# richardbaihe/a3t

Hardware: AMD Instinct MI355X
Metric: mel-frames/sec (train) (higher is better)
Workload: dtype bf16; 1 GPU; VCTK A3T masked-mel train step: 6+6 Conformer blocks d=384 H=2 ff=1536(k3), B=32/GPU, T_mel=1000, T_phn=120, postnet 5x256x5, fwd+bwd+clip+Adam, dropout 0.2/0.2/0.2 + postnet 0.5 (recipe); global_batch=32, parallelism=dp1, params=100799808

## Files before the change

### a3t_amd/_lib.py

```python
import ctypes
import os
from ctypes import POINTER, c_char_p, c_float, c_int, c_int32, c_int64, c_void_p

import torch

HERE = os.path.dirname(os.path.abspath(__file__))
LIB_PATH = os.environ.get("A3T_LIB_PATH") or os.path.join(HERE, "lib", "liba3t_hip.so")

F32, BF16 = 0, 1
BF16X3 = 2
ACT_NONE, ACT_RELU, ACT_TANH, ACT_SWISH = 0, 1, 2, 3
ACC_STORE, ACC_ADD, ACC_ATOMIC, ACC_SOLE = 0, 1, 2, 3


class GemmDesc(ctypes.Structure):
    _fields_ = [
        ("A", c_void_p), ("B", c_void_p), ("C", c_void_p), ("bias", c_void_p), ("R", c_void_p), ("S", c_void_p),
        ("M", c_int32), ("N", c_int32), ("K", c_int32),
        ("a_rs", c_int64), ("a_cs", c_int64),
        ("b_rs", c_int64), ("b_cs", c_int64), ("b_ts", c_int64),
        ("c_rs", c_int64),
        ("batch", c_int32), ("batch_inner", c_int32),
        ("a_bs0", c_int64), ("a_bs1", c_int64), ("b_bs0", c_int64), ("b_bs1", c_int64),
        ("c_bs0", c_int64), ("c_bs1", c_int64),
        ("taps", c_int32), ("pad", c_int32), ("dil", c_int32), ("Tseq", c_int32), ("kshift", c_int32),
        ("alpha", c_float),
        ("act", c_int32), ("accumulate", c_int32), ("splitk", c_int32),
        ("a_dtype", c_int32), ("b_dtype", c_int32), ("c_dtype", c_int32), ("compute", c_int32),
        ("s_dtype", c_int32), ("colsum_slots", c_int32),
        ("colsum", c_void_p), ("colsum_bs1", c_int64), ("colsum_scale", c_float), ("drop_key", ctypes.c_uint32),
        ("drop_p", c_float), ("colsum_ss", c_int32),
        ("keep_out", c_void_p), ("keep_in", c_void_p),
        ("a_signmask", c_int32), ("keep_layout", c_int32),
        ("A2", c_void_p), ("B2", c_void_p), ("b2_cs", c_int64), ("b2_bs0", c_int64), ("b2_bs1", c_int64), ("colsum2", c_void_p),
        ("a2_rs", c_int64), ("a_unaligned", c_int32),
    ]


_P = c_void_p
_SIGS = {
    "a3t_gemm": [POINTER(GemmDesc), _P],
    "a3t_gemm_plan": [POINTER(GemmDesc), c_char_p, c_int],
    "a3t_layernorm_fwd": [_P, _P, _P, _P, c_int, _P, _P, c_int, c_int, c_float, _P],
    "a3t_layernorm_bwd": [_P, c_int, _P, _P, _P, _P, _P, _P, _P, _P, _P, _P, c_float, c_int, c_int, c_float,
                          ctypes.c_uint32, _P],
    "a3t_col_reduce": [_P, c_int, _P, _P, _P, _P, c_int, c_int, c_int64, c_int, _P],
    "a3t_f64_to_f32_add": [_P, _P, c_int, c_float, _P],
    "a3t_bn_act_fwd": [_P, _P, _P, _P, _P, _P, _P, _P, _P, c_int, c_int, c_int, c_float, c_float, c_int, c_int, _P],
    "a3t_bn_act_bwd_a": [_P, c_int, _P, _P, _P, _P, _P, _P, c_int, c_int, c_int, _P],
    "a3t_bn_act_bwd_b": [_P, c_int, _P, _P, _P, _P, _P, _P, _P, _P, _P, c_int, c_int, c_int, c_int, _P],
    "a3t_glu_dwconv_fwd": [_P, c_int, _P, _P, _P, c_int, _P, c_int, c_int, c_int, c_int, _P],
    "a3t_glu_dwconv_bwd": [_P, _P, c_int, _P, c_int, _P, _P, c_int, _P, _P, _P, c_int, c_int, c_int, c_int, _P],
    "a3t_add_pos_bias": [_P, _P, _P, _P, _P, c_int, c_int, c_int, _P],
    "a3t_add_pos_bias_bwd": [_P, _P, _P, c_int, c_int, c_int, _P],
    "a3t_relpos_softmax_fwd": [_P, _P, c_int, _P, _P, c_int, c_int, c_int, c_int, c_int64, c_int64, c_int64, c_float, _P,
                               c_float, ctypes.c_uint32, _P],
    "a3t_relpos_softmax_bwd": [_P, c_int, _P, c_int, _P, _P, c_int, c_int, c_int, c_int, c_int64, c_int64, c_int64, c_float, _P,
                               c_float, c_int64, c_int64, ctypes.c_uint32, _P, _P],
    "a3t_attn_fwd_train": [_P, _P, _P, _P, _P, _P, _P, _P, _P, _P, _P, c_int, c_int, c_int, c_int, c_int64, c_int64, c_int64,
                           c_int64, c_float, c_float, ctypes.c_uint32, _P, _P, _P],
    "a3t_attn_scale_rows": [_P, _P, _P, c_int, c_int, c_int, c_int, _P],
    "a3t_attn_bwd_ds": [_P, _P, _P, _P, _P, _P, _P, c_int, c_int, c_int, c_int, c_int64, c_int64, c_int64, c_int64, c_float,
                        c_float, ctypes.c_uint32, c_int, c_int64, _P],
    "a3t_attn_fwd": [_P, _P, _P, _P, _P, _P, _P, _P, c_int, c_int, c_int, c_int, c_int64, c_int64, c_int64, c_int64,
                     c_float, c_float, ctypes.c_uint32, _P, _P, _P],
    "a3t_pwg_block": [_P, _P, _P, _P, _P, _P, _P, _P, c_int, c_int, c_int, _P],
    "a3t_mask_fill": [_P, _P, _P, _P, c_int, c_int, c_int, _P],
    "a3t_embed_finish_fwd": [_P, _P, _P, _P, _P, _P, _P, c_int, c_int, c_int, c_int, c_float, c_float, ctypes.c_uint32,
                             _P, _P],
    "a3t_embed_finish_bwd": [_P, _P, _P, _P, _P, _P, _P, _P, c_int, c_int, c_int, c_int, c_int, c_int, c_float, c_float,
                             ctypes.c_uint32, _P],
    "a3t_scale": [_P, _P, c_int64, c_float, _P],
    "a3t_attn_fwd_plain": [_P, _P, _P, _P, _P, _P, c_int, c_int, c_int, c_int, c_int64, c_int64, c_int64, c_float, c_float,
                           ctypes.c_uint32, _P],
    "a3t_attn_fwd_train_plain": [_P, _P, _P, _P, _P, _P, _P, _P, _P, c_int, c_int, c_int, c_int, c_int64, c_int64, c_int64, c_float,
                                 c_float, ctypes.c_uint32, _P],
    "a3t_embed_finish_abs_fwd": [_P, _P, _P, _P, _P, _P, _P, _P, _P, _P, c_int, c_int, c_int, c_int, c_float, c_float,
                                 ctypes.c_uint32, _P, _P],
    "a3t_embed_finish_abs_bwd": [_P, _P, _P, _P, _P, _P, _P, _P, _P, _P, _P, _P, c_int, c_int, c_int, c_int, c_int, c_int,
                                 c_float, c_float, ctypes.c_uint32, _P],
    "a3t_embed_finish_abs_partials": [c_int, c_int, c_int, c_int],
    "a3t_scale_add_pos": [_P, _P, _P, c_int, c_int, c_int, c_float, c_float, ctypes.c_uint32, _P],
    "a3t_softmax_plain_fwd": [_P, c_int, _P, _P, c_int, c_int, c_int, c_int, c_int64, c_int64, c_float, _P, c_float,
                              ctypes.c_uint32, _P],
    "a3t_softmax_plain_bwd": [_P, c_int, _P, c_int, _P, c_int, c_int, c_int, c_int, c_int64, c_int64, c_int64, c_float, _P,
                              c_float, ctypes.c_uint32, _P, _P],
    "a3t_axpy": [_P, _P, c_int64, c_float, _P],
    "a3t_attn_bias_fold": [_P, c_int32, c_int32, _P, _P, _P, _P],
    "a3t_scale_dev": [_P, _P, c_int64, _P, _P],
    "a3t_slice_rows": [_P, _P, c_int, c_int, c_int, c_int, c_int, c_int, _P],
    "a3t_concat_rows": [_P, _P, _P, c_int, c_int, c_int, c_int, _P],
    "a3t_concat_rows_ragged": [_P, _P, _P, _P, _P, c_int, c_int, c_int, c_int, c_int64, c_int64, _P],
    "a3t_split_rows": [_P, _P, _P, c_int, c_int, c_int, c_int, _P],
    "a3t_cast_bf16": [_P, _P, c_int64, _P],
    "a3t_cast_bf16_conv_t": [_P, _P, _P, _P, c_int, c_int, c_int, c_int, _P],
    "a3t_split_bf16": [_P, _P, _P, c_int64, _P],
    "a3t_reflect_pad": [_P, _P, c_int, c_int, c_int, c_int, _P],
    "a3t_reflect_pad_ragged": [_P, _P, _P, c_int, c_int, c_int, c_int, _P],
    "a3t_stft_amp": [_P, _P, c_int64, c_int, c_int, _P],
    "a3t_logmel_finish": [_P, _P, c_int, c_int, c_int, _P],
    "a3t_mlm_loss": [_P, _P, _P, _P, _P, _P, _P, _P, c_int, c_int, c_int, c_float, _P],
    "a3t_mlm_loss_scratch_floats": [c_int],
    "a3t_sumsq": [_P, c_int64, _P, _P],
    "a3t_clip_adam": [_P, _P, _P, _P, _P, _P, c_int64, c_float, c_float, c_float, c_float, c_int, c_float, c_float,
                      _P],
    "a3t_clip_adam_noam": [_P, _P, _P, _P, _P, _P, c_int64, _P, c_float, c_float, c_float, c_float, c_float, c_float,
                           c_float, c_float, _P],
    "a3t_sgd_step": [_P, _P, c_int64, c_float, c_float, _P],
    "a3t_pwg_gate": [_P, _P, _P, c_int64, c_int, _P],
    "a3t_pwg_res_skip": [_P, _P, _P, c_int64, c_int, c_int, _P],
    "a3t_pwg_upsample": [_P, _P, _P, c_int64, c_int64, c_int, c_int, _P],
    "a3t_replicate_pad": [_P, _P, c_int64, c_int64, c_int, c_int, _P],
    "a3t_bias_act": [_P, _P, c_int64, c_int, c_int, c_float, _P],
    "a3t_replicate_pad_ragged": [_P, _P, _P, c_int64, c_int64, c_int, c_int, _P],
    "a3t_pwg_upsample_ragged": [_P, _P, _P, _P, c_int, c_int64, c_int64, c_int, c_int, _P],
    "a3t_zero_tail": [_P, _P, c_int, c_int64, c_int64, c_int, _P],
# ... 83 lines not shown
```

### a3t_amd/build.py

```python
import os
import subprocess
import sys
from concurrent.futures import ThreadPoolExecutor

HERE = os.path.dirname(os.path.abspath(__file__))
CSRC = os.path.join(HERE, "csrc")
LIBDIR = os.path.join(HERE, "lib")
LIB = os.path.join(LIBDIR, "liba3t_hip.so")
SOURCES = ["gemm.hip", "gemm_bf16.hip", "gemm_bf16_8p.hip", "gemm_bf16_tn.hip", "gemm_bf16_pn.hip", "gemm_bf16_tt.hip", "attn_fused.hip", "norm_reduce.hip", "convmod_attn.hip", "dwconv_vec.hip", "misc.hip", "pwg_fused.hip", "pwg_fused_f16.hip", "features.hip", "duration.hip", "fs2_tts.hip", "gst.hip", "hifigan.hip", "hifigan_f16.hip", "melgan.hip", "stylemelgan.hip"]
FLAGS = ["--offload-arch=gfx950", "-O3", "-std=c++17", "-fPIC", "-ffp-contract=off"] + os.environ.get("A3T_EXTRA_FLAGS", "").split()


WAVE_SOURCES = ("pwg_fused.hip", "pwg_fused_f16.hip", "hifigan.hip", "hifigan_f16.hip", "melgan.hip", "stylemelgan.hip")
RES_SOURCES = ("gemm_bf16.hip", "gemm_bf16_8p.hip", "gemm_bf16_tn.hip", "gemm_bf16_pn.hip", "gemm_bf16_tt.hip", "attn_fused.hip", "norm_reduce.hip") + WAVE_SOURCES
RES_FLAG = ["-Rpass-analysis=kernel-resource-usage"]


def _save_resources(report, path):
    import json
    import re
    cur, rows = None, {}
    for ln in report.splitlines():
        m = re.search(r"Function Name: (\S+)", ln)
        if m:
            cur = m.group(1)
            rows[cur] = {}
            continue
        m = re.search(r"remark:\s+([\w \[\]/]+?): (\d+)", ln)
        if m and cur:
            rows[cur][m.group(1).strip()] = int(m.group(2))
    with open(path, "w") as f:
        json.dump(rows, f, indent=1)


def _hipcc():
    for c in ("/opt/rocm/bin/hipcc", "hipcc"):
        if os.path.exists(c) or c == "hipcc":
            return c


def _stale(out, deps):
    if not os.path.exists(out):
        return True
    t = os.path.getmtime(out)
    return any(os.path.getmtime(d) > t for d in deps)


def build(force=False, verbose=True):
    os.makedirs(LIBDIR, exist_ok=True)
    hdrs = [os.path.join(os.path.dirname(HERE), "include", "a3t_hip.h")]
    hdrs += sorted(os.path.join(CSRC, h) for h in os.listdir(CSRC) if h.endswith(".h"))
    objs, jobs = [], []
    for s in SOURCES:
        src = os.path.join(CSRC, s)
        obj = os.path.join(LIBDIR, s.replace(".hip", ".o"))
        objs.append(obj)
        if force or _stale(obj, [src] + hdrs):
            jobs.append([_hipcc(), *FLAGS, "-c", src, "-o", obj] + (RES_FLAG if s in RES_SOURCES else []))

    def run(cmd):
        if verbose:
            print(" ".join(cmd), flush=True)
        if RES_FLAG[0] in cmd:
            r = subprocess.run(cmd, stderr=subprocess.PIPE, text=True)
            if r.returncode:
                sys.stderr.write(r.stderr)
                raise subprocess.CalledProcessError(r.returncode, cmd)
# ... 15 lines not shown
```

### a3t_amd/conformer.py

```python
import math
import os
import zlib
from dataclasses import dataclass

import torch

from . import ops
from ._lib import ACC_ADD, ACC_ATOMIC, ACC_STORE, ACT_RELU, ACT_SWISH, BF16, BF16X3, F32
from .config import A3TConfig
from .params import ParamStore
from .schedule import StepSchedule


def legacy_pe_table(c: A3TConfig) -> torch.Tensor:
    d = c.adim
    position = torch.arange(c.max_len - 1, -1, -1.0, dtype=torch.float32).unsqueeze(1)
    div = torch.exp(torch.arange(0, d, 2, dtype=torch.float32) * -(math.log(10000.0) / d))
    pe = torch.zeros(c.max_len, d)
    pe[:, 0::2] = torch.sin(position * div)
    pe[:, 1::2] = torch.cos(position * div)
    return pe


def score_chunks(lengths, heads, max_score_elems):
# ... 447 lines not shown
        if rs is not None:
            dctx_v = self._act(self._t("tmp.dctxs"), (M, d))
        signed = bool(self.sv.get(tag + ".signed"))
        adr = self._drop(c.attention_dropout_rate, tag + ".att") if (pdrop is not None or signed) else None
        regen = self.bf16 and adr is not None and T % 8 == 0 and T <= 2048
        ds_fused = (rs is not None and self.bf16 and self.opt.attn_bwd_ds and (adr is None or regen) and dk % 32 == 0 and dk <= 192
                    and dk != 160 and T % 8 == 0)
        zb = (H * T * T, T * T)
        assert ds_fused or not signed
        if not ds_fused:
            dpr = self.ws.get("tmp.ac", (B, H, T, T), sdt)
            ops.gemm(dctx, vv, dpr, T, T, dk, d, 1, 3 * d, 1, T, batch=B * H, batch_inner=H, a_bs=(T * d, dk),
                     b_bs=(T * 3 * d, dk), c_bs=zb, compute=cmp)
        fz = self.bf16
        gbq = gr[pre + ".bqkv"]
        S = self.colsum_slots
        sl = self._arena_slot("bwd32", tag + ".bsl", S * 4 * d) if fz else None
        csk = dict(colsum_bs1=dk, colsum_slots=S, colsum_ss=4 * d)
        make_q = qu is None
        if make_q:
            qu = self._act("tmp.qu", (M, d))
            qv = self._act(self._t("tmp.qv"), (M, d))

        def dv_gemm():
            if rs is not None:
                ops.attn_scale_rows(dctx, rs, dctx_v, B, H, T)
            ops.gemm(pdrop if pdrop is not None else probs, dctx_v, dvv, T, dk, T, 1, T, 1, d, 3 * d,
                     batch=B * H, batch_inner=H, a_bs=zb, b_bs=(T * d, dk), c_bs=(T * 3 * d, dk),
                     compute=cmp, colsum=sl[3 * d:] if fz else None, a_signmask=signed,
                     alpha=1.0 / (1.0 - adr[0]) if signed else 1.0, **csk)
            if make_q:
                ops.add_pos_bias(qkv, p[pre + ".u"], p[pre + ".v"], qu, qv)
        qv_ready = self._side(dv_gemm, want_event=make_q, urgent=True)
        zbd = zb
        dual = ds_fused and fz and self.opt.attn_dq_dual and ops.gemm_tt_supported(T, dk, T, B * H)
        dview = ds_fused and fz and self.opt.attn_dbd_view
        if dview:
            bsv = T + T * T
            flat = self.ws.get(self._t("tmp.dsv"), (B * H * bsv,), torch.bfloat16, zero_once=True)
            ds, dbd = flat[T:], flat[1:]
            zbd = (H * bsv, bsv)
        elif self.bf16:
            ds = self.ws.get("tmp.ds16", (B, H, T, T), torch.bfloat16)
            dbd = self.ws.get(self._t("tmp.dbd16"), (B, H, T, T), torch.bfloat16)
        else:
            ds = dpr
            dbd = self.ws.get(self._t("tmp.dbd"), (B, H, T, T), sdt)
        if ds_fused:
            ops.attn_bwd_ds(dctx, ctx, qkv, probs, rs, ds, None if dview else dbd, B, H, T, scale, drop=adr or (0.0, 0),
                            signed_probs=signed, ds_bs=zbd[1] if dview else 0)
        else:
            ops.relpos_softmax_bwd(probs, dpr, ds, dbd, B, H, T, scale, probs_drop=None if regen else pdrop,
                                   drop_p=adr[0] if adr else 0.0, drop_key=adr[1] if regen else 0, rowscale=rs)
        def pos_weight_grad():
            if qv_ready is not None and self.side is not None:
                qv_ready.wait_on(self.side)
            dP = self._arena_slot("bwd32", tag + ".dP", T * d).view(T, d)
            ops.gemm(dbd, qv, dP, T, dk, T, 1, T + 1 if dview else T, 1, d, d, batch=B * H, batch_inner=H, a_bs=zbd, b_bs=(T * d, dk),
                     c_bs=(0, dk), acc=ACC_ATOMIC, compute=cmp, a_view=dview)
            if self.bf16:
                dP16 = self.ws.get("tmp.dP16", (T, d), torch.bfloat16)
                ops.cast_bf16(dP, dP16)
                dP = dP16
            ops.linear_bwd_weight(dP, pos, gr[pre + ".wpos"], compute=cmp)
        self._side(pos_weight_grad)
        dq_acc = fz
        dqu = dqkv if dq_acc else self._act("tmp.dqu", (M, d))
        dqv = dqkv if dq_acc else self._act("tmp.dqv", (M, d))
        ldq, cbq = (3 * d, (T * 3 * d, dk)) if dq_acc else (d, (T * d, dk))
        if dual:
            ops.gemm(ds, kk, dqkv, T, dk, T, T, 1, 1, 3 * d, ldq, batch=B * H, batch_inner=H, a_bs=zbd,
                     b_bs=(T * 3 * d, dk), c_bs=cbq, compute=cmp, colsum=sl,
                     second=(dbd, P, d, (0, dk), sl[d:]) + ((T + 1,) if dview else ()), **csk)
        else:
            ops.gemm(ds, kk, dqu, T, dk, T, T, 1, 1, 3 * d, ldq, batch=B * H, batch_inner=H, a_bs=zbd,
                     b_bs=(T * 3 * d, dk), c_bs=cbq, compute=cmp, colsum=sl if fz else None, **csk)
        dk_fn = lambda: ops.gemm(ds, qu, dkk, T, dk, T, 1, T, 1, d, 3 * d, batch=B * H, batch_inner=H,
                                 a_bs=zbd, b_bs=(T * d, dk), c_bs=(T * 3 * d, dk), compute=cmp,
                                 colsum=sl[2 * d:] if fz else None, **csk)
        if self.opt.attn_dk_main and dual and self.side is not None and make_q and qv_ready is not None:
            qv_ready.wait_on(torch.cuda.current_stream())
            dk_fn()
            dk_done = None
        else:
            dk_done = self._side(dk_fn, want_event=True, urgent=True)
        if not dual:
            ops.gemm(dbd, P, dqv, T, dk, T, T + 1 if dview else T, 1, 1, d, ldq, batch=B * H, batch_inner=H, a_bs=zbd, b_bs=(0, dk),
                     c_bs=cbq, acc=ACC_ADD if dq_acc else ACC_STORE, compute=cmp, colsum=sl[d:] if fz else None, a_view=dview, **csk)
        if not dq_acc:
            ops.add_pos_bias_bwd(dqu, dqv, dqkv)
        if dk_done is not None:
            dk_done.wait_on(torch.cuda.current_stream())
        if fz:
            self._side(
                lambda: ops.attn_bias_fold(sl, S, d, gr[pre + ".u"], gr[pre + ".v"], gbq))
        else:
            self._bias_grad(dqu, gr[pre + ".u"])
            self._bias_grad(dqv, gr[pre + ".v"])
            self._bias_grad(dqkv, gbq)
        self._lin_wgrad(dqkv, y, gr[pre + ".wqkv"])
        dy = self._act("tmp.dy", (M, d))
        self._lin_dgrad(dqkv, pre + ".wqkv", dy)
        self._pre_ln(ga, g, g16)
        self._ln_bwd(tag + ".ln", dy, pre + ".ln", g, g, g16, nb, nxt)
        self._sub_end()
        return g

    def _bn_fwd(self, tag, z, pre, bufpre, act, out):
        p, b = self.store.p, self.store.buf
# ... 210 lines not shown
```

### a3t_amd/ops.py

```python
import ctypes
import os

import torch

from . import _lib as L
from ._lib import ACC_ADD, ACC_ATOMIC, ACC_SOLE, ACC_STORE, ACT_NONE, ACT_RELU, ACT_SWISH, ACT_TANH, BF16, F32

__all__ = ["gemm", "gemm_plan", "linear_fwd", "linear_bwd_data", "linear_bwd_weight", "conv_fwd", "conv_bwd_data",
           "conv_bwd_weight"]


PROFILE = None


def _stream():
    return ctypes.c_void_p(torch.cuda.current_stream().cuda_stream)


def _ptr(t):
    if t is None:
        return None
    return ctypes.c_void_p(t.data_ptr())


# ... 321 lines not shown
    dk = d // H
    kk = qkv.view(-1)[d:]
    vv = qkv.view(-1)[2 * d:]
    pqu, pqv, ldq, pbu, pbv = _attn_q_operands(qu, qv, qkv, pos_bias)
    e0 = None
    if PROFILE is not None:
        e0, e1 = torch.cuda.Event(enable_timing=True), torch.cuda.Event(enable_timing=True)
        e0.record()
    L.check(L.load().a3t_attn_fwd_train(pqu, pqv, _ptr(kk), _ptr(vv), _ptr(P), _ptr(keymask), _ptr(ctx), _ptr(lse),
                                        _ptr(probs), _ptr(probs_drop), _ptr(rowscale), B, H, T, dk, ldq, 3 * d, d, d, scale,
                                        drop[0], drop[1], pbu, pbv, _stream()), "attn_fwd_train")
    if e0 is not None:
        e1.record()
        PROFILE.append((f"attn_fwd32_kernel<{dk // 32}, {'true' if drop[0] > 0 else 'false'}, true, false, false, {'true' if (drop[0] > 0 and probs_drop is None) else 'false'}>", 3 * 2.0 * B * H * T * T * dk, e0, e1,
                        (T, T, dk, B * H, 1, 1)))


def attn_fwd_plain(qkv, keymask, ctx, lse, B, H, T, scale, drop=(0.0, 0)):
    d = qkv.shape[1] // 3
    if qkv.dtype != torch.bfloat16 or ctx.dtype != torch.bfloat16 or qkv.shape[0] < B * T or ctx.numel() < B * T * d or \
            lse.numel() < B * H * T or keymask.numel() < B * T or d % H:
        raise ValueError("attn_fwd_plain: shapes do not fit")
    L.check(L.load().a3t_attn_fwd_plain(_ptr(qkv), _ptr(qkv.view(-1)[d:]), _ptr(qkv.view(-1)[2 * d:]), _ptr(keymask), _ptr(ctx),
                                        _ptr(lse), B, H, T, d // H, 3 * d, 3 * d, d, scale, drop[0], drop[1], _stream()),
            "attn_fwd_plain")


def attn_fwd_train_plain(qkv, keymask, ctx, lse, probs, probs_drop, rowscale, B, H, T, scale, drop=(0.0, 0)):
    d = qkv.shape[1] // 3
    n = B * H * T * T
    if qkv.dtype != torch.bfloat16 or ctx.dtype != torch.bfloat16 or probs.dtype != torch.bfloat16 or qkv.shape[0] < B * T or \
            ctx.numel() < B * T * d or lse.numel() < B * H * T or rowscale.numel() < B * H * T or keymask.numel() < B * T or \
            probs.numel() < n or (probs_drop is not None and (probs_drop.numel() < n or probs_drop.dtype != torch.bfloat16)) or d % H:
        raise ValueError("attn_fwd_train_plain: shapes do not fit")
    L.check(L.load().a3t_attn_fwd_train_plain(_ptr(qkv), _ptr(qkv.view(-1)[d:]), _ptr(qkv.view(-1)[2 * d:]), _ptr(keymask),
                                              _ptr(ctx), _ptr(lse), _ptr(probs), _ptr(probs_drop), _ptr(rowscale), B, H, T, d // H,
                                              3 * d, 3 * d, d, scale, drop[0], drop[1], _stream()), "attn_fwd_train_plain")


def attn_scale_rows(x, rowscale, y, B, H, T):
    d = x.shape[1]
    L.check(L.load().a3t_attn_scale_rows(_ptr(x), _ptr(rowscale), _ptr(y), B, H, T, d // H, _stream()), "attn_scale_rows")


def attn_bwd_ds(dctx, ctx, qkv, probs, rowscale, ds, dbd, B, H, T, scale, drop=(0.0, 0), dbd_head_major=False, signed_probs=False,
                ds_bs=0):
    d = dctx.shape[1]
    v = qkv.view(-1)[2 * d:]
    bsb, bsh = ((T * T, B * T * T) if dbd_head_major else (0, 0))
    L.check(L.load().a3t_attn_bwd_ds(_ptr(dctx), _ptr(ctx), _ptr(v), _ptr(probs), _ptr(rowscale), _ptr(ds), _ptr(dbd), B, H, T,
                                     d // H, d, 3 * d, bsb, bsh, scale, drop[0], drop[1], 1 if signed_probs else 0, ds_bs, _stream()), "attn_bwd_ds")


def mask_fill(speech, masked, mask_feature, out):
    M, C = out.shape
    L.check(L.load().a3t_mask_fill(_ptr(speech), _ptr(masked), _ptr(mask_feature), _ptr(out), _dt(out), M, C,
                                   _stream()), "mask_fill")


def embed_finish_fwd(e, emb, seg, text, spos, tpos, xs, B, Tm, Tp, D, xscale, drop=(0.0, 0), spk=None):
    L.check(L.load().a3t_embed_finish_fwd(_ptr(e), _ptr(emb), _ptr(seg), _ptr(text), _ptr(spos), _ptr(tpos), _ptr(xs),
                                          B, Tm, Tp, D, xscale, drop[0], drop[1], _ptr(spk), _stream()), "embed_fwd")


def embed_finish_bwd(dxs, e, text, spos, tpos, de, demb, dseg, B, Tm, Tp, D, V, nseg, xscale, drop=(0.0, 0)):
    L.check(L.load().a3t_embed_finish_bwd(_ptr(dxs), _ptr(e), _ptr(text), _ptr(spos), _ptr(tpos), _ptr(de),
                                          _ptr(demb), _ptr(dseg), B, Tm, Tp, D, V, nseg, xscale, drop[0], drop[1],
                                          _stream()), "embed_bwd")


def _f32c(t, n, what):
    if t is None or t.dtype != torch.float32 or not t.is_contiguous() or t.numel() < n:
        raise ValueError(f"{what}: expected a contiguous float32 tensor of >= {n} elements")
    return t


def embed_finish_abs_fwd(e, emb, seg, text, spos, tpos, pe, alpha, xs, B, Tm, Tp, D, xscale, drop=(0.0, 0), spk=None):
    _f32c(pe, max(Tm, Tp) * D, "pe")
    _f32c(xs, B * (Tm + Tp) * D, "xs")
    if Tm:
        _f32c(e, B * Tm * D, "e")
    if Tp and (text.dtype != torch.int64 or text.numel() < B * Tp):
        raise ValueError("text: expected int64 [B][Tp]")
    if seg is not None and (spos.numel() < B * Tm or tpos.numel() < B * Tp or spos.dtype != torch.int64 or tpos.dtype != torch.int64):
        raise ValueError("spos / tpos: expected int64 [B][Tm] / [B][Tp]")
    a_s, a_t = alpha if alpha is not None else (None, None)
    L.check(L.load().a3t_embed_finish_abs_fwd(_ptr(e), _ptr(emb), _ptr(seg), _ptr(text), _ptr(spos), _ptr(tpos), _ptr(pe),
                                              _ptr(a_s), _ptr(a_t), _ptr(xs), B, Tm, Tp, D, xscale, drop[0], drop[1], _ptr(spk),
                                              _stream()), "embed_abs_fwd")


def embed_finish_abs_partials(B, Tm, Tp, D):
    return int(L.load().a3t_embed_finish_abs_partials(B, Tm, Tp, D))


def embed_finish_abs_bwd(dxs, e, text, spos, tpos, pe, de, demb, dseg, dalpha, partial, B, Tm, Tp, D, V, nseg, xscale,
                         drop=(0.0, 0)):
    _f32c(pe, max(Tm, Tp) * D, "pe")
    _f32c(dxs, B * (Tm + Tp) * D, "dxs")
    if Tm:
        _f32c(e, B * Tm * D, "e")
        _f32c(de, B * Tm * D, "de")
    if Tp:
        _f32c(demb, V * D, "demb")
    d_s, d_t = dalpha if dalpha is not None else (None, None)
    if dalpha is not None:
# ... 594 lines not shown
```

### include/a3t_hip.h

```cpp
#ifndef A3T_HIP_H
#define A3T_HIP_H
#include <stdint.h>

#ifdef __cplusplus
extern "C" {
#endif

#define A3T_F32 0
#define A3T_BF16 1
#define A3T_BF16X3 2

#define A3T_EINVAL (-22)

#define A3T_ACT_NONE 0
#define A3T_ACT_RELU 1
#define A3T_ACT_TANH 2
#define A3T_ACT_SWISH 3

#define A3T_ACC_STORE 0
#define A3T_ACC_ADD 1
#define A3T_ACC_ATOMIC 2
#define A3T_ACC_SOLE 3

typedef struct a3t_gemm_desc {
// ... 54 lines not shown
                   double* out1, int M, int C, int64_t ld, int mode, void* stream);
int a3t_f64_to_f32_add(const double* src, float* dst, int n, float scale, void* stream);

int a3t_bn_act_fwd(const float* z, const double* stats, const float* gamma, const float* beta,
                   float* running_mean, float* running_var, float* mean_out, float* rstd_out, void* y,
                   int y_dtype, int M, int C, float eps, float momentum, int training, int act, void* stream);
int a3t_bn_act_bwd_a(const void* dy, int dy_dtype, const float* z, const float* mean, const float* rstd,
                     const float* gamma, const float* beta, double* sums, int M, int C, int act, void* stream);
int a3t_bn_act_bwd_b(const void* dy, int dy_dtype, const float* z, const float* mean, const float* rstd,
                     const float* gamma, const float* beta, const double* sums, float* dz, float* dgamma,
                     float* dbeta, int M, int C, int training, int act, void* stream);

int a3t_glu_dwconv_fwd(const void* g, int g_dtype, const float* wdw, const float* bdw, void* glu,
                       int glu_dtype, float* z, int M, int C, int K, int Tseq, void* stream);
int a3t_glu_dwconv_bwd(const float* dz, const void* g, int g_dtype, const void* glu, int glu_dtype,
                       const float* wdw, void* dg, int dg_dtype, float* dwdw, float* dbdw, float* dg_colsum,
                       int M, int C, int K, int Tseq, void* stream);

int a3t_add_pos_bias(const void* qkv, const float* bias_u, const float* bias_v, void* qu, void* qv, int dtype,
                     int M, int d, void* stream);
int a3t_add_pos_bias_bwd(const void* dqu, const void* dqv, void* dqkv, int dtype, int M, int d, void* stream);
int a3t_relpos_softmax_fwd(const void* ac, const void* bd, int scores_dtype, const uint8_t* keymask, void* probs,
                           int probs_dtype, int B, int H, int T, int64_t ac_bs, int64_t bd_bs, int64_t p_bs,
                           float scale, void* probs_drop, float drop_p, uint32_t drop_key, void* stream);
int a3t_relpos_softmax_bwd(const void* probs, int probs_dtype, const void* dprobs, int dprobs_dtype, void* ds,
                           void* dbd, int out_dtype, int B, int H, int T, int64_t p_bs, int64_t dp_bs, int64_t o_bs,
                           float scale, const void* probs_drop, float drop_p, int64_t dbd_bs_b, int64_t dbd_bs_h,
                           uint32_t drop_key, const float* rowscale, void* stream);
int a3t_softmax_plain_fwd(const void* ac, int scores_dtype, const uint8_t* keymask, void* probs, int probs_dtype, int B, int H,
                          int T, int64_t ac_bs, int64_t p_bs, float scale, void* probs_drop, float drop_p, uint32_t drop_key,
                          void* stream);
int a3t_softmax_plain_bwd(const void* probs, int probs_dtype, const void* dprobs, int dprobs_dtype, void* ds, int out_dtype,
                          int B, int H, int T, int64_t p_bs, int64_t dp_bs, int64_t o_bs, float scale, const void* probs_drop,
                          float drop_p, uint32_t drop_key, const float* rowscale, void* stream);

int a3t_attn_fwd(const void* qu, const void* qv, const void* k, const void* v, const void* pos, const uint8_t* keymask,
                 void* ctx, float* lse, int B, int H, int T, int dk, int64_t ldq, int64_t ldkv, int64_t ldp, int64_t ldo,
                 float scale, float drop_p, uint32_t drop_key, const float* bias_u, const float* bias_v, void* stream);

int a3t_attn_fwd_train(const void* qu, const void* qv, const void* k, const void* v, const void* pos,
                       const uint8_t* keymask, void* ctx, float* lse, void* probs, void* probs_drop, float* rowscale,
                       int B, int H, int T, int dk, int64_t ldq, int64_t ldkv, int64_t ldp, int64_t ldo, float scale,
                       float drop_p, uint32_t drop_key, const float* bias_u, const float* bias_v, void* stream);
int a3t_attn_fwd_plain(const void* q, const void* k, const void* v, const uint8_t* keymask, void* ctx, float* lse, int B, int H,
                       int T, int dk, int64_t ldq, int64_t ldkv, int64_t ldo, float scale, float drop_p, uint32_t drop_key,
                       void* stream);
int a3t_attn_fwd_train_plain(const void* q, const void* k, const void* v, const uint8_t* keymask, void* ctx, float* lse, void* probs,
                             void* probs_drop, float* rowscale, int B, int H, int T, int dk, int64_t ldq, int64_t ldkv,
                             int64_t ldo, float scale, float drop_p, uint32_t drop_key, void* stream);
int a3t_attn_scale_rows(const void* x, const float* rowscale, void* y, int B, int H, int T, int dk, void* stream);
int a3t_attn_bwd_ds(const void* dctx, const void* ctx, const void* v, const void* probs, const float* rowscale, void* ds,
                    void* dbd, int B, int H, int T, int dk, int64_t ldo, int64_t ldkv, int64_t dbd_bsb, int64_t dbd_bsh,
                    float scale, float drop_p, uint32_t drop_key, int signed_probs, int64_t ds_bs, void* stream);

int a3t_mask_fill(const float* speech, const uint8_t* masked, const float* mask_feature, void* out,
                  int out_dtype, int M, int C, void* stream);
int a3t_embed_finish_fwd(const float* e, const float* emb, const float* seg, const int64_t* text,
                         const int64_t* spos, const int64_t* tpos, float* xs, int B, int Tm, int Tp, int D,
                         float xscale, float drop_p, uint32_t drop_key, const float* spk, void* stream);
int a3t_embed_finish_bwd(const float* dxs, const float* e, const int64_t* text, const int64_t* spos,
                         const int64_t* tpos, float* de, float* demb, float* dseg, int B, int Tm, int Tp,
                         int D, int V, int nseg, float xscale, float drop_p, uint32_t drop_key, void* stream);
int a3t_embed_finish_abs_fwd(const float* e, const float* emb, const float* seg, const int64_t* text, const int64_t* spos,
                             const int64_t* tpos, const float* pe, const float* alpha_s, const float* alpha_t, float* xs, int B,
                             int Tm, int Tp, int D, float xscale, float drop_p, uint32_t drop_key, const float* spk,
                             void* stream);
int a3t_embed_finish_abs_bwd(const float* dxs, const float* e, const int64_t* text, const int64_t* spos, const int64_t* tpos,
                             const float* pe, float* de, float* demb, float* dseg, float* dalpha_s, float* dalpha_t,
                             float* partial, int B, int Tm, int Tp, int D, int V, int nseg, float xscale, float drop_p,
                             uint32_t drop_key, void* stream);
int a3t_embed_finish_abs_partials(int B, int Tm, int Tp, int D);
int a3t_scale_add_pos(const float* x, const float* pe, float* y, int B, int T, int D, float s, float drop_p, uint32_t drop_key,
                      void* stream);
int a3t_scale(const float* x, float* y, int64_t n, float s, void* stream);
int a3t_axpy(const float* x, float* y, int64_t n, float a, void* stream);
int a3t_attn_bias_fold(const float* slots, int S, int d, float* gu, float* gv, float* gbqkv, void* stream);
int a3t_scale_dev(const float* x, float* y, int64_t n, const float* s, void* stream);
int a3t_slice_rows(const float* x, void* y, int y_dtype, int B, int T, int Tm, int D, int reverse_add,
                   void* stream);
int a3t_concat_rows(const float* speech, const float* text, float* xs, int B, int Tm, int Tp, int D, void* stream);
int a3t_split_rows(const float* dxs, float* dspeech, float* dtext, int B, int Tm, int Tp, int D, void* stream);
int a3t_concat_rows_ragged(const float* speech, const float* text, float* xs, const int32_t* slens, const int32_t* tlens, int B,
                           int Tm, int Tp, int D, int64_t speech_bs, int64_t text_bs, void* stream);
int a3t_cast_bf16(const float* x, void* y, int64_t n, void* stream);
int a3t_cast_bf16_conv_t(const float* src, void* dst, const int64_t* src_off, const int64_t* dst_off, int count, int N,
                         int taps, int C, void* stream);
int a3t_split_bf16(const float* x, void* hi, void* lo, int64_t n, void* stream);

int a3t_reflect_pad(const float* x, float* out, int B, int N, int pad, int ld, void* stream);
int a3t_reflect_pad_ragged(const float* x, float* out, const int32_t* lens, int B, int N, int pad, int ld, void* stream);
int a3t_stft_amp(const float* S, float* amp, int64_t rows, int nbins, int ld, void* stream);
int a3t_logmel_finish(float* mel, const int64_t* olens, int B, int F, int C, void* stream);

int a3t_mlm_loss(const float* before, const float* after, const float* target, const uint8_t* masked,
                 float* loss_out, float* d_before, float* d_after, float* scratch, int M, int C, int l2,
                 float gscale, void* stream);
int a3t_mlm_loss_scratch_floats(int M);

int a3t_sumsq(const float* g, int64_t n, double* partial , void* stream);
int a3t_clip_adam(float* p, const float* g, float* m, float* v, const double* partial, float* norm_out,
                  int64_t n, float lr, float beta1, float beta2, float eps, int step, float clip,
                  float gscale, void* stream);

int a3t_clip_adam_noam(float* p, const float* g, float* m, float* v, const double* partial, float* norm_out, int64_t n,
                       int32_t* state, float base_lr, float model_size, float warmup, float beta1, float beta2,
                       float eps, float clip, float gscale, void* stream);
// ... 109 lines not shown
```

Measured before the change: 818,200 mel-frames/s.

## Add streaming MFMA kernel for relpos position-gradient with batch-grouped partial sums

Replaces the batched atomic-accumulate GEMM that computes dP = sum over batch/heads of dbd^T·qv with a dedicated kernel. Each workgroup owns a row tile and head, streams K-tiles across a group of batch items through a multi-stage LDS pipeline filled by async DMA, and accumulates in registers. It writes per-group fp32 partials that a fold kernel reduces to a bf16 dP. This avoids fp32 atomics and the fp32 arena round trip, but adds a workspace buffer and an extra fold launch, and the fold changes the summation order.

```diff
diff --git a/a3t_amd/_lib.py b/a3t_amd/_lib.py
--- a/a3t_amd/_lib.py
+++ b/a3t_amd/_lib.py
@@ -62,6 +62,9 @@
     "a3t_attn_scale_rows": [_P, _P, _P, c_int, c_int, c_int, c_int, _P],
     "a3t_attn_bwd_ds": [_P, _P, _P, _P, _P, _P, _P, c_int, c_int, c_int, c_int, c_int64, c_int64, c_int64, c_int64, c_float,
                         c_float, ctypes.c_uint32, c_int, c_int64, _P],
+    "a3t_attn_bwd_dpos": [_P, _P, _P, _P, _P, c_int, c_int, c_int, c_int, c_int64, c_int64, c_int64, _P],
+    "a3t_attn_bwd_dpos_ws": [c_int, c_int, c_int, c_int],
+    "a3t_attn_bwd_dpos_plan": [c_int, c_int, c_int, c_int, POINTER(c_int)],
     "a3t_attn_fwd": [_P, _P, _P, _P, _P, _P, _P, _P, c_int, c_int, c_int, c_int, c_int64, c_int64, c_int64, c_int64,
                      c_float, c_float, ctypes.c_uint32, _P, _P, _P],
     "a3t_pwg_block": [_P, _P, _P, _P, _P, _P, _P, _P, c_int, c_int, c_int, _P],
diff --git a/a3t_amd/build.py b/a3t_amd/build.py
--- a/a3t_amd/build.py
+++ b/a3t_amd/build.py
@@ -7,12 +7,12 @@
 CSRC = os.path.join(HERE, "csrc")
 LIBDIR = os.path.join(HERE, "lib")
 LIB = os.path.join(LIBDIR, "liba3t_hip.so")
-SOURCES = ["gemm.hip", "gemm_bf16.hip", "gemm_bf16_8p.hip", "gemm_bf16_tn.hip", "gemm_bf16_pn.hip", "gemm_bf16_tt.hip", "attn_fused.hip", "norm_reduce.hip", "convmod_attn.hip", "dwconv_vec.hip", "misc.hip", "pwg_fused.hip", "pwg_fused_f16.hip", "features.hip", "duration.hip", "fs2_tts.hip", "gst.hip", "hifigan.hip", "hifigan_f16.hip", "melgan.hip", "stylemelgan.hip"]
+SOURCES = ["gemm.hip", "gemm_bf16.hip", "gemm_bf16_8p.hip", "gemm_bf16_tn.hip", "gemm_bf16_pn.hip", "gemm_bf16_tt.hip", "attn_fused.hip", "attn_dpos.hip", "norm_reduce.hip", "convmod_attn.hip", "dwconv_vec.hip", "misc.hip", "pwg_fused.hip", "pwg_fused_f16.hip", "features.hip", "duration.hip", "fs2_tts.hip", "gst.hip", "hifigan.hip", "hifigan_f16.hip", "melgan.hip", "stylemelgan.hip"]
 FLAGS = ["--offload-arch=gfx950", "-O3", "-std=c++17", "-fPIC", "-ffp-contract=off"] + os.environ.get("A3T_EXTRA_FLAGS", "").split()
 
 
 WAVE_SOURCES = ("pwg_fused.hip", "pwg_fused_f16.hip", "hifigan.hip", "hifigan_f16.hip", "melgan.hip", "stylemelgan.hip")
-RES_SOURCES = ("gemm_bf16.hip", "gemm_bf16_8p.hip", "gemm_bf16_tn.hip", "gemm_bf16_pn.hip", "gemm_bf16_tt.hip", "attn_fused.hip", "norm_reduce.hip") + WAVE_SOURCES
+RES_SOURCES = ("gemm_bf16.hip", "gemm_bf16_8p.hip", "gemm_bf16_tn.hip", "gemm_bf16_pn.hip", "gemm_bf16_tt.hip", "attn_fused.hip", "attn_dpos.hip", "norm_reduce.hip") + WAVE_SOURCES
 RES_FLAG = ["-Rpass-analysis=kernel-resource-usage"]
 
 
diff --git a/a3t_amd/conformer.py b/a3t_amd/conformer.py
--- a/a3t_amd/conformer.py
+++ b/a3t_amd/conformer.py
@@ -523,9 +523,17 @@
         else:
             ops.relpos_softmax_bwd(probs, dpr, ds, dbd, B, H, T, scale, probs_drop=None if regen else pdrop,
                                    drop_p=adr[0] if adr else 0.0, drop_key=adr[1] if regen else 0, rowscale=rs)
+        dpos = self.bf16 and dbd.dtype == torch.bfloat16 and ops.attn_bwd_dpos_plan(B, H, T, dk) is not None
+        dpos_ws = self.ws.get(self._t("tmp.dPws"), (ops.attn_bwd_dpos_ws(B, H, T, dk),)) if dpos else None
+
         def pos_weight_grad():
             if qv_ready is not None and self.side is not None:
                 qv_ready.wait_on(self.side)
+            if dpos:
+                dP16 = self.ws.get("tmp.dP16", (T, d), torch.bfloat16)
+                ops.attn_bwd_dpos(dbd, qv, dpos_ws, dP16, B, H, T, T + 1 if dview else T, zbd)
+                ops.linear_bwd_weight(dP16, pos, gr[pre + ".wpos"], compute=cmp)
+                return
             dP = self._arena_slot("bwd32", tag + ".dP", T * d).view(T, d)
             ops.gemm(dbd, qv, dP, T, dk, T, 1, T + 1 if dview else T, 1, d, d, batch=B * H, batch_inner=H, a_bs=zbd, b_bs=(T * d, dk),
                      c_bs=(0, dk), acc=ACC_ATOMIC, compute=cmp, a_view=dview)
diff --git a/a3t_amd/csrc/attn_dpos.hip b/a3t_amd/csrc/attn_dpos.hip
--- /dev/null
+++ b/a3t_amd/csrc/attn_dpos.hip
@@ -0,0 +1,236 @@
+#include <hip/hip_runtime.h>
+#include <stdint.h>
+#include "../../include/a3t_hip.h"
+#include "dtype_io.h"
+#include "device_cus.h"
+#include "mfma_kit.h"
+
+typedef short s16x4 __attribute__((ext_vector_type(4)));
+typedef short s16x8 __attribute__((ext_vector_type(8)));
+typedef unsigned short u16;
+
+#ifndef DPOS_NPA
+#define DPOS_NPA 3
+#endif
+#ifndef DPOS_STAGES
+#define DPOS_STAGES 6
+#endif
+
+namespace {
+constexpr int DP_NPA = DPOS_NPA, DP_STAGES = DPOS_STAGES, DP_BK = 32;
+constexpr int DP_MAX_ROWS = 64 * DP_NPA;
+constexpr int DP_Q = (4 * (DP_NPA + 3) + 7) / 8;
+constexpr int DP_WA = 4 * DP_NPA / DP_Q;
+constexpr int DP_A_BYTES = DP_NPA * 4096, DP_STAGE = 8 * DP_Q * 1024, DP_LDS = DP_STAGES * DP_STAGE;
+static_assert(DP_WA * DP_Q == 4 * DP_NPA && (8 - DP_WA) * DP_Q >= 12, "a wave requests A pieces or B pieces, never both");
+static_assert(DP_STAGE - DP_A_BYTES >= 3 * 4096, "three B panels behind the A panels");
+static_assert(DP_LDS <= 160 * 1024 && DP_STAGES >= 4 && DP_Q * (DP_STAGES - 1) < 64, "LDS of a CU; the vmcnt field");
+
+struct DposArgs {
+    const u16* dbd;
+    const u16* qv;
+    float* ws;
+    int B, H, T, dk, d;
+    int64_t a_rs, a_bsb, a_bsh;
+    int TR, ntiles, G;
+};
+
+template <int N>
+__device__ __forceinline__ void wait_vm() {
+    asm volatile("s_waitcnt vmcnt(%0)" ::"n"(N) : "memory");
+}
+
+template <int NJ, int NPA, int STAGES>
+__global__ __launch_bounds__(512) void attn_dpos_stream_kernel(DposArgs p) {
+    extern __shared__ __attribute__((aligned(16))) unsigned char smem[];
+    constexpr int NBI = 2 * NPA;
+    const int tid = threadIdx.x, lane = tid & 63;
+    const int w = __builtin_amdgcn_readfirstlane(tid >> 6);
+    const int wr = w >> 2, wc = w & 3;
+    const int wi = xcd_contiguous(blockIdx.x, gridDim.x);
+    const int tm = wi % p.ntiles, zz = wi / p.ntiles;
+    const int h = zz % p.H, grp = zz / p.H;
+    const int b0 = grp * p.G;
+    const int nb = min(p.G, p.B - b0);
+    const int T = p.T, TR = p.TR, dk = p.dk;
+    const int m0 = tm * TR;
+    const int nbi = TR >> 5;
+    const int nkt = (T + DP_BK - 1) / DP_BK;
+    const int nkt_all = nb * nkt;
+
+    const bool is_a = w < DP_WA;
+    const unsigned a_ld = (unsigned)p.a_rs * 2u, b_ld = (unsigned)p.d * 2u;
+    const unsigned ld = is_a ? a_ld : b_ld;
+    const unsigned ext = is_a ? (unsigned)(T - 1) * a_ld + (unsigned)T * 2u : (unsigned)(T - 1) * b_ld + (unsigned)dk * 2u;
+    const u16* X0 = is_a ? p.dbd + h * p.a_bsh : p.qv + h * dk;
+    const int64_t xbs = is_a ? p.a_bsb : (int64_t)T * p.d;
+    const unsigned lds0 = __builtin_amdgcn_readfirstlane((unsigned)(uintptr_t)LDS_AS(smem));
+
+    unsigned voff[DP_Q];
+    int kq[DP_Q];
+#pragma unroll
+    for (int q = 0; q < DP_Q; ++q) {
+        const int s = (is_a ? w : w - DP_WA) * DP_Q + q;
+        const int r = (s & 3) * 8 + (lane >> 3);
+        const int sw = ((r >> 1) & 1) | (((r >> 3) & 1) << 1);
+        const int col = (s >> 2) * 64 + (((lane & 7) ^ (sw << 1)) << 3);
+        const bool ok = is_a ? (col < TR && m0 + col < T) : (col < dk && col < 64 * NJ);
+        voff[q] = ok ? (unsigned)r * ld + (unsigned)((is_a ? m0 : 0) + col) * 2u : OOB;
+        kq[q] = r;
+    }
+    const unsigned kstep = 32u * ld;
+    const unsigned dst0 = lds0 + (is_a ? (unsigned)(w * DP_Q) * 1024u : (unsigned)DP_A_BYTES + (unsigned)((w - DP_WA) * DP_Q) * 1024u);
+    int ik = 0, ib = 0, si = 0;
+    auto issue = [&]() __attribute__((always_inline)) {
+        const unsigned dst = dst0 + (unsigned)si * (unsigned)DP_STAGE;
+        const bool live = ib < nb;
+        const __amdgpu_buffer_rsrc_t rX = __builtin_amdgcn_make_buffer_rsrc((void*)(X0 + (int64_t)(b0 + (live ? ib : 0)) * xbs), 0, (int)ext, 0x00020000);
+        const unsigned so = live ? (unsigned)ik * kstep : 0u;
+        const int krem = live ? T - ik * DP_BK : 0;
+#pragma unroll
+        for (int q = 0; q < DP_Q; ++q) dma16(rX, dst + q * 1024, kq[q] < krem ? voff[q] : OOB, so);
+        si = si + 1 == STAGES ? 0 : si + 1;
+        if (++ik == nkt) ik = 0, ++ib;
+    };
+
+    const int g = lane >> 4, pp = lane & 15;
+    const unsigned swr = (unsigned)((((pp >> 3) & 1) | ((g & 1) << 1)) << 1);
+    const unsigned kbyte = (unsigned)(g * 8 + (pp >> 2)) * 128u + (unsigned)(pp & 1) * 8u;
+    auto frag_rc = [&](const unsigned char* img, const int c0) __attribute__((always_inline)) -> bf16x8 {
+        const unsigned cb = (unsigned)((c0 & 63) >> 3) + (unsigned)((pp >> 1) & 1);
+        const unsigned char* a0 = img + (c0 >> 6) * 4096 + kbyte + ((cb ^ swr) << 4);
+        s16x4 lo = __builtin_amdgcn_ds_read_tr16_b64_v4i16((__attribute__((address_space(3))) s16x4*)LDS_AS(a0));
+        s16x4 hi = __builtin_amdgcn_ds_read_tr16_b64_v4i16((__attribute__((address_space(3))) s16x4*)LDS_AS(a0 + 512));
+        s16x8 v = {lo[0], lo[1], lo[2], lo[3], hi[0], hi[1], hi[2], hi[3]};
+        return __builtin_bit_cast(bf16x8, v);
+    };
+
+    f32x4 acc[NBI][NJ];
+#pragma unroll
+    for (int i = 0; i < NBI; ++i)
+#pragma unroll
+        for (int j = 0; j < NJ; ++j) acc[i][j] = f32x4{0.f, 0.f, 0.f, 0.f};
+
+#pragma unroll
+    for (int s = 0; s < STAGES - 1; ++s) issue();
+    const int rb0 = wr * nbi;
+    int sr = 0;
+    for (int kt = 0; kt < nkt_all; ++kt) {
+        wait_vm<DP_Q*(STAGES - 2)>();
+        BAR();
+        issue();
+        const unsigned char* sA = smem + sr * DP_STAGE;
+        const unsigned char* sB = sA + DP_A_BYTES;
+        sr = sr + 1 == STAGES ? 0 : sr + 1;
+        bf16x8 fb[NJ];
+#pragma unroll
+        for (int j = 0; j < NJ; ++j) fb[j] = frag_rc(sB, wc * (16 * NJ) + j * 16);
+        bf16x8 fa[NBI];
+#pragma unroll
+        for (int i = 0; i < NBI; ++i) fa[i] = frag_rc(sA, (rb0 + i) * 16);
+        SB();
+#pragma unroll
+        for (int i = 0; i < NBI; ++i)
+#pragma unroll
+            for (int j = 0; j < NJ; ++j) acc[i][j] = __builtin_amdgcn_mfma_f32_16x16x32_bf16(fb[j], fa[i], acc[i][j], 0, 0, 0);
+    }
+    wait_vm<0>();
+    __syncthreads();
+
+    const int crow = m0 + rb0 * 16 + pp;
+    const int ccol = wc * (16 * NJ) + g * 4;
+    float* W = p.ws + (int64_t)grp * T * p.d + h * dk + ccol;
+#pragma unroll
+    for (int i = 0; i < NBI; ++i) {
+        const int row = crow + i * 16;
+        const bool rok = i < nbi && row < T;
+#pragma unroll
+        for (int j = 0; j < NJ; ++j)
+            if (rok && ccol + j * 16 < dk) *(f32x4*)(W + (int64_t)row * p.d + j * 16) = acc[i][j];
+    }
+}
+
+__global__ __launch_bounds__(256) void attn_dpos_fold_kernel(const float* __restrict__ ws, u16* __restrict__ dP16, float* __restrict__ dP,
+                                                             int groups, int64_t n) {
+    const int64_t i = ((int64_t)blockIdx.x * 256 + threadIdx.x) * 8;
+    if (i >= n) return;
+    float4 a = *(const float4*)(ws + i), b = *(const float4*)(ws + i + 4);
+    for (int g = 1; g < groups; ++g) {
+        const float4 u = *(const float4*)(ws + g * n + i), v = *(const float4*)(ws + g * n + i + 4);
+        a.x += u.x, a.y += u.y, a.z += u.z, a.w += u.w;
+        b.x += v.x, b.y += v.y, b.z += v.z, b.w += v.w;
+    }
+    uint4 o;
+    o.x = io_pack2(a.x, a.y), o.y = io_pack2(a.z, a.w), o.z = io_pack2(b.x, b.y), o.w = io_pack2(b.z, b.w);
+    *(uint4*)(dP16 + i) = o;
+    if (dP) *(float4*)(dP + i) = a, *(float4*)(dP + i + 4) = b;
+}
+
+struct DposPlan {
+    int rows, tiles, group, grid, groups;
+};
+
+bool dpos_plan(int B, int H, int T, int dk, DposPlan* pl) {
+    if (B < 1 || H < 1 || T < 8 || T % 8 || dk < 32 || dk % 32 || dk > 192 || dk == 160) return false;
+    const int64_t d = (int64_t)H * dk;
+    if ((int64_t)(T - 1) * (T + 1) * 2 + (int64_t)T * 2 >= (1ll << 31) || (int64_t)T * d * 2 >= (1ll << 31)) return false;
+    const int cus = device_cus();
+    int tiles = 0, tr = 0, G = 0;
+    long best = 0;
+    for (int t = (T + DP_MAX_ROWS - 1) / DP_MAX_ROWS, n = 0; n < 6; ++t, ++n) {
+        const int r = (((T + t - 1) / t) + 31) / 32 * 32;
+        if (r > DP_MAX_ROWS || (int64_t)r * (t - 1) >= T || (int64_t)t * H > cus) continue;
+        const int maxg = cus / (t * H), gg = (B + maxg - 1) / maxg;
+        const long cost = (long)gg * (r + 64);
+        if (!tiles || cost < best) tiles = t, tr = r, G = gg, best = cost;
+    }
+    if (!tiles) return false;
+    const int64_t units = (int64_t)tiles * H;
+    const int groups = (B + G - 1) / G;
+    if ((int64_t)groups * T * d >= (1ll << 31)) return false;
+    pl->rows = tr, pl->tiles = tiles, pl->group = G, pl->groups = groups, pl->grid = (int)(units * groups);
+    return true;
+}
+
+template <int NJ>
+void launch_stream(const DposArgs& a, int grid, hipStream_t stream) {
+    (void)hipFuncSetAttribute((const void*)attn_dpos_stream_kernel<NJ, DP_NPA, DP_STAGES>, hipFuncAttributeMaxDynamicSharedMemorySize, DP_LDS);
+    hipLaunchKernelGGL((attn_dpos_stream_kernel<NJ, DP_NPA, DP_STAGES>), dim3(grid), dim3(512), DP_LDS, stream, a);
+}
+}
+
+extern "C" int a3t_attn_bwd_dpos_plan(int B, int H, int T, int dk, int* out) {
+    DposPlan pl;
+    if (!dpos_plan(B, H, T, dk, &pl)) return 0;
+    if (out) out[0] = pl.rows, out[1] = pl.tiles, out[2] = pl.group, out[3] = pl.grid;
+    return 1;
+}
+
+extern "C" int a3t_attn_bwd_dpos_ws(int B, int H, int T, int dk) {
+    DposPlan pl;
+    if (!dpos_plan(B, H, T, dk, &pl)) return 0;
+    return (int)((int64_t)pl.groups * T * H * dk);
+}
+
+extern "C" int a3t_attn_bwd_dpos(const void* dbd, const void* qv, float* ws, void* dP16, float* dP, int B, int H, int T, int dk,
+                                 int64_t dbd_rs, int64_t dbd_bsb, int64_t dbd_bsh, void* stream) {
+    DposPlan pl;
+    if (!dbd || !qv || !ws || !dP16 || !dpos_plan(B, H, T, dk, &pl)) return A3T_EINVAL;
+    if (((uintptr_t)dbd & 1) || ((uintptr_t)qv & 15) || ((uintptr_t)ws & 15) || ((uintptr_t)dP16 & 15) || ((uintptr_t)dP & 15)) return A3T_EINVAL;
+    if (dbd_rs < T || dbd_bsb < 0 || dbd_bsh < 0 || (dbd_rs * (int64_t)(T - 1) + T) * 2 >= (1ll << 31)) return A3T_EINVAL;
+    DposArgs a;
+    a.dbd = (const u16*)dbd, a.qv = (const u16*)qv, a.ws = ws;
+    a.B = B, a.H = H, a.T = T, a.dk = dk, a.d = H * dk;
+    a.a_rs = dbd_rs, a.a_bsb = dbd_bsb, a.a_bsh = dbd_bsh;
+    a.TR = pl.rows, a.ntiles = pl.tiles, a.G = pl.group;
+    if (dk > 128)
+        launch_stream<3>(a, pl.grid, (hipStream_t)stream);
+    else
+        launch_stream<2>(a, pl.grid, (hipStream_t)stream);
+    int rc = (int)hipGetLastError();
+    if (rc) return rc;
+    const int64_t n = (int64_t)T * a.d;
+    hipLaunchKernelGGL(attn_dpos_fold_kernel, dim3((unsigned)((n / 8 + 255) / 256)), dim3(256), 0, (hipStream_t)stream, (const float*)ws,
+                       (u16*)dP16, dP, pl.groups, n);
+    return (int)hipGetLastError();
+}
diff --git a/a3t_amd/ops.py b/a3t_amd/ops.py
--- a/a3t_amd/ops.py
+++ b/a3t_amd/ops.py
@@ -397,6 +397,23 @@
                                      d // H, d, 3 * d, bsb, bsh, scale, drop[0], drop[1], 1 if signed_probs else 0, ds_bs, _stream()), "attn_bwd_ds")
 
 
+def attn_bwd_dpos_plan(B, H, T, dk):
+    out = (ctypes.c_int * 4)()
+    if not L.load().a3t_attn_bwd_dpos_plan(int(B), int(H), int(T), int(dk), out):
+        return None
+    return tuple(out)
+
+
+def attn_bwd_dpos_ws(B, H, T, dk):
+    return int(L.load().a3t_attn_bwd_dpos_ws(int(B), int(H), int(T), int(dk)))
+
+
+def attn_bwd_dpos(dbd, qv, ws, dP16, B, H, T, dbd_rs, dbd_bs, dP=None):
+    d = qv.shape[1]
+    L.check(L.load().a3t_attn_bwd_dpos(_ptr(dbd), _ptr(qv), _ptr(ws), _ptr(dP16), _ptr(dP), B, H, T, d // H, int(dbd_rs),
+                                       int(dbd_bs[0]), int(dbd_bs[1]), _stream()), "attn_bwd_dpos")
+
+
 def mask_fill(speech, masked, mask_feature, out):
     M, C = out.shape
     L.check(L.load().a3t_mask_fill(_ptr(speech), _ptr(masked), _ptr(mask_feature), _ptr(out), _dt(out), M, C,
diff --git a/include/a3t_hip.h b/include/a3t_hip.h
--- a/include/a3t_hip.h
+++ b/include/a3t_hip.h
@@ -130,6 +130,10 @@
 int a3t_attn_bwd_ds(const void* dctx, const void* ctx, const void* v, const void* probs, const float* rowscale, void* ds,
                     void* dbd, int B, int H, int T, int dk, int64_t ldo, int64_t ldkv, int64_t dbd_bsb, int64_t dbd_bsh,
                     float scale, float drop_p, uint32_t drop_key, int signed_probs, int64_t ds_bs, void* stream);
+int a3t_attn_bwd_dpos(const void* dbd, const void* qv, float* ws, void* dP16, float* dP, int B, int H, int T, int dk, int64_t dbd_rs,
+                      int64_t dbd_bsb, int64_t dbd_bsh, void* stream);
+int a3t_attn_bwd_dpos_ws(int B, int H, int T, int dk);
+int a3t_attn_bwd_dpos_plan(int B, int H, int T, int dk, int* out);
 
 int a3t_mask_fill(const float* speech, const uint8_t* masked, const float* mask_feature, void* out,
                   int out_dtype, int M, int C, void* stream);
```

Result: faster. 829,400 mel-frames/s (median of 6 runs) (+1.4%).
